# Da-Tsuchi/KLab_MultiModalModel

Measured on AMD Instinct MI355X. Metric: caption-train samples/sec (224px img, 64-tok tgt), higher is better.
Workload: dtype bf16; 1 GPU; BASELINE configs[1]: Swin-V2(C=64,(2,2,6,2),224,w7) frozen + T5-small, fwd+bwd+Adam, T5 dropout 0.1 on, random-init weights; global_batch=64, per_gpu_batch=64, src_len=9, tgt_len=64, parallelism=dp1, hipgraph=False, optimizer=klab.optim.FusedAdam (Adam update of ref/train.py:28, one kernel)

## Files before the change

include/klab_mm.h:

```cpp
#ifndef KLAB_MM_H
#define KLAB_MM_H
#include <stddef.h>
#include <stdint.h>

#ifdef __cplusplus
extern "C" {
#endif

#define KLAB_OK 0
#define KLAB_ERR_UNSUPPORTED (-2)
#define KLAB_ERR_BADARG (-3)

#define KLAB_F32 0
#define KLAB_BF16 1
#define KLAB_FP8 2

#define KLAB_ACT_NONE 0
#define KLAB_ACT_RELU 1
#define KLAB_ACT_GELU 2

#define KLAB_AUX_NONE 0
#define KLAB_AUX_NONZERO 1
#define KLAB_AUX_DGELU 2

// ... 122 lines not shown

#define KLAB_JPEG_GRAY 0
#define KLAB_JPEG_YCC 1
#define KLAB_JPEG_RGB 2
typedef struct klab_jpeg_info {
  int width, height, ncomp, precision, progressive, supported, colour;
  int hmax, vmax, mcus_x, mcus_y;
  int hs[3], vs[3], bw[3], bh[3], tq[3];
  long long coef_blocks;
} klab_jpeg_info;
typedef struct klab_jpeg_item { klab_jpeg_info info; long long coef_block0; long long rgb_off; } klab_jpeg_item;
int klab_jpeg_read_info(const unsigned char* data, size_t n, klab_jpeg_info* info);
int klab_jpeg_entropy_decode(const unsigned char* data, size_t n, short* coefs, unsigned short* qt, klab_jpeg_info* info);
int klab_jpeg_entropy_decode_batch(const unsigned char* const* data, const size_t* sizes, int n, short* const* coefs,
                                   unsigned short* qt, klab_jpeg_info* infos, int* rcs, int n_threads);
size_t klab_jpeg_decode_ws_bytes(const klab_jpeg_item* items, int n);
int klab_jpeg_decode_device(const short* coefs_dev, const unsigned short* qt_dev, const klab_jpeg_item* items,
                            const klab_jpeg_item* items_dev, int n, unsigned char* rgb_dev, void* ws, size_t ws_bytes, void* stream);

int klab_cast_pack(const void* desc_dev, int ndesc, long total4, void* dst, int dtype, void* stream);
int klab_embed_fwd(const long long* ids, int shift_right, int L, int start_id, int pad_id, const float* table, int vocab,
                   float* out, int rows, int d, float drop_p, const uint32_t* seed_dev, uint32_t tag, int* err_flag,
                   void* stream);
int klab_embed_bwd(const long long* ids, int shift_right, int L, int start_id, int pad_id, const float* dh, float* dtable,
                   int vocab, int rows, int d, float drop_p, const uint32_t* seed_dev, uint32_t tag, void* stream);
int klab_relbias_fwd(const float* table, const int* bucket, float* bias, int heads, int Lq, int Lk, void* stream);
int klab_relbias_bwd(const float* dbias, const int* bucket, float* dtable, int heads, int Lq, int Lk, int nbuckets,
                     void* stream);
int klab_ce_count(const long long* labels, int rows, float* inv_n, void* stream);
int klab_ce_fwd(void* logits, long ld, int dtype, const long long* labels, int rows, int V, float* inv_n, float* loss_row,
                float* loss, int write_grad, void* stream);
int klab_im2col_patch(const float* pixels, void* out, int dtype, int B, int Cin, int Himg, int P, void* stream);
int klab_im2col_patch_ld(const float* pixels, void* out, int dtype, int B, int Cin, int Himg, int P, int ldo, void* stream);
int klab_merge_gather(const float* x, void* out, int dtype, int B, int R, int C, void* stream);
int klab_merge_scatter(const float* dmerged, float* dx, int B, int R, int C, void* stream);
int klab_colsum(const void* dy, long ld, int dtype, int M, int N, float* out, void* stream);
int klab_convert(const float* x, void* y, int dtype, long n, float scale, void* stream);
int klab_add_f32(float* y, const float* x, long n, void* stream);

int klab_gelu_fwd(const void* x, void* y, int dtype, long n, void* stream);
int klab_geglu_fwd(const void* ab, long ldab, void* h, long ldh, int dtype, int M, int F, float drop_p, const uint32_t* seed_dev,
                   uint32_t drop_tag, void* stream);
int klab_geglu_bwd(const void* dh, long lddh, const void* ab, long ldab, void* dab, long lddab, int dtype, int M, int F, float drop_p,
                   const uint32_t* seed_dev, uint32_t drop_tag, void* stream);
int klab_swin_proj_ln_fused(const void* x, const float* shortcut, const void* w, const float* b, const float* gamma, const float* beta,
                            float* out, void* outt, int dtype, int M, int C, float eps, void* stream);
int klab_swin_mlp_fused(const void* x, const float* shortcut, const void* w1, const float* b1, const void* w2, const float* b2,
                        const float* gamma, const float* beta, float* out, void* outt, int dtype, int M, int C, float eps,
                        void* stream);
int klab_swin_patch_embed_fused(const float* pixels, const void* w, int ldw, const float* bias, const float* gamma, const float* beta,
                                float* out, void* outt, int dtype, int B, int in_ch, int image_size, int patch, int C, float eps, void* stream);
int klab_swin_linear_ln_fused(const void* x, const float* shortcut, const void* w, const float* bias, const float* gamma,
                              const float* beta, float* out, void* outt, int dtype, int M, int K, int C, float eps, void* stream);
int klab_swin_cpb_bias_bwd(const float* dbias, const float* bias, const int* index, const float* coords, const float* hidden,
                           const float* w0, const float* w2, float* dtable, float* dw0, float* db0, float* dw2, int ntab, int n,
                           int heads, int nhidden, void* stream);
int klab_swin_cpb_bias_bwd_pz(const float* dbias, const float* bias, const int* index, const float* coords, const float* hidden,
                              const float* w0, const float* w2, float* dtable, float* dw0, float* db0, float* dw2, int ntab, int n,
                              int heads, int nhidden, int dtable_zeroed, void* stream);

typedef struct klab_swin_cfg {
  int image_size, patch, in_ch, embed_dim, n_stages;
  int depths[8], heads[8];
  int window;
  int pretrained_window[8];
  int mlp_ratio, qkv_bias;
  float ln_eps;
} klab_swin_cfg;
typedef struct klab_t5_cfg {
  int vocab, d_model, d_kv, n_heads, d_ff, n_layers, n_dec_layers, rel_buckets, rel_max_dist;
  float dropout, ln_eps;
  int start_id, pad_id, scale_decoder_outputs;
  int ffn_gated;
  int tie_lm_head;
} klab_t5_cfg;
typedef struct klab_model_cfg {
  klab_swin_cfg swin;
  klab_t5_cfg lang, main;
  int dtype;
  int train_swin;
} klab_model_cfg;
typedef struct klab_engine klab_engine;

int klab_sizeof_t5_cfg(void);
int klab_sizeof_model_cfg(void);
int klab_sizeof_sample_args(void);
int klab_sizeof_logits_proc_args(void);
int klab_sizeof_gen_cfg(void);
klab_engine* klab_engine_create(const klab_model_cfg* cfg);
void klab_engine_destroy(klab_engine* e);
int klab_engine_num_params(const klab_engine* e, int model);
int klab_engine_param_info(const klab_engine* e, int model, int i, char* name, int name_cap, long* shape4, int* ndim,
                           long* grad_off );
long klab_engine_grad_elems(const klab_engine* e, int model);
int klab_engine_num_buckets(const klab_engine* e, int segment);
int klab_engine_bucket(const klab_engine* e, int segment, int i, long* off, long* len);
int klab_engine_bucket_wait(klab_engine* e, int segment, int i, void* stream);
int klab_engine_set_bucket_events(klab_engine* e, int on);
int klab_engine_segment(const klab_engine* e, int seg, int* model, long* off, long* len);
size_t klab_engine_workspace_bytes(klab_engine* e, int B, int Ls, int Lt);
int klab_engine_bind(klab_engine* e, int B, int Ls, int Lt, void* workspace, size_t ws_bytes, const void* const* swin_params,
                     const void* const* lang_params, const void* const* main_params, float* main_grads, float* swin_grads,
                     const int* lang_bucket, const int* enc_bucket, const int* dec_bucket, const void* const* swin_coords,
                     const void* const* swin_index, void* stream);
int klab_engine_forward(klab_engine* e, const float* pixels, const long long* src_ids, const long long* tgt_ids, int training,
                        uint32_t seed, int want_grad, void* stream);
// ... 118 lines not shown
```

klab_multimodalmodel_amd/_lib.py:

```python
import ctypes as C
import os

HERE = os.path.dirname(os.path.abspath(__file__))
LIB_PATH = os.environ.get("KLAB_LIB", os.path.join(HERE, "libklab_mm.so"))

F32, BF16, FP8 = 0, 1, 2
ACT_NONE, ACT_RELU, ACT_GELU = 0, 1, 2
AUX_NONE, AUX_NONZERO, AUX_DGELU = 0, 1, 2
ERR_UNSUPPORTED, ERR_BADARG = -2, -3

vp, i32, i64, f32, u32 = C.c_void_p, C.c_int, C.c_long, C.c_float, C.c_uint32


class GemmArgs(C.Structure):
    _fields_ = [("M", i32), ("N", i32), ("K", i32), ("dtype", i32),
                ("A", vp), ("lda", i64), ("a_kmajor", i32),
                ("B", vp), ("ldb", i64), ("b_kmajor", i32),
                ("C", vp), ("ldc", i64), ("c_dtype", i32), ("accumulate", i32),
                ("alpha", f32), ("alpha_dev", vp), ("bias", vp), ("act", i32),
                ("aux", vp), ("ldaux", i64), ("aux_mode", i32), ("aux_scale", f32),
                ("residual", vp), ("ldr", i64), ("r_dtype", i32),
                ("drop_p", f32), ("seed_dev", vp), ("drop_tag", u32), ("name_tag", i32), ("atomic_ok", i32)]


# ... 59 lines not shown
class GenCfg(C.Structure):
    _fields_ = [("mode", i32), ("n", i32), ("max_length", i32), ("eos_id", i32), ("pad_id", i32),
                ("temperature", f32), ("top_k", i32), ("top_p", f32), ("seed", C.c_uint64),
                ("length_penalty", f32), ("early_stopping", i32), ("procs", C.POINTER(LogitsProcCfg)), ("want_logprobs", i32)]


SIGNATURES = {
    "klab_version": [],
    "klab_gemm": [C.POINTER(GemmArgs), vp],
    "klab_gemm_probe_enable": [i32],
    "klab_gemm_probe_read": [vp, vp, vp],
    "klab_rmsnorm_fwd": [vp, vp, vp, i32, vp, vp, i32, i32, f32, i32, i32, i32, f32, vp, u32, vp],
    "klab_rmsnorm_bwd": [vp, vp, vp, vp, vp, vp, vp, i32, vp, i32, i32, i32, i32, i32, f32, u32, f32, u32, vp, vp],
    "klab_rmsnorm_bwd_part": [vp, vp, vp, vp, vp, vp, vp, i32, vp, i32, i32, i32, i32, i32, f32, u32, f32, u32, vp, vp],
    "klab_rmsnorm_part_rows": [i32],
    "klab_colpart_reduce": [vp, i64, i32, i32, vp, i32, vp],
    "klab_adam_step": [vp, i32, i64, vp, vp, vp, vp, i32, f32, f32, f32, f32, f32, f32, f32, vp],
    "klab_adam_step_range": [vp, i32, i64, i64, vp, vp, vp, vp, i32, f32, f32, f32, f32, f32, f32, f32, vp],
    "klab_adafactor_plan": [i32, vp, vp, vp, vp, vp],
    "klab_adafactor_step": [vp, i32, i64, i64, vp, vp, vp, vp, vp, vp, i32, f32, f32, f32, f32, f32, f32, f32, f32, f32, i32, vp],
    "klab_layernorm_fwd": [vp, i32, vp, vp, vp, vp, vp, i32, vp, vp, i32, i32, f32, i32, i32, i32, f32, vp, u32, vp],
    "klab_layernorm_bwd": [vp, vp, i32, vp, vp, vp, vp, vp, vp, i32, i32, i32, i32, i32, f32, vp, u32, vp],
    "klab_rmsnorm_fwd_q8": [vp, vp, vp, vp, vp, vp, i32, i32, f32, f32, vp, u32, vp],
    "klab_layernorm_fwd_q8": [vp, vp, vp, vp, vp, vp, vp, vp, vp, vp, i32, i32, f32, vp],
    "klab_gelu_fwd": [vp, vp, i32, i64, vp],
    "klab_gelu_fwd_q8": [vp, vp, vp, vp, i32, i32, vp],
    "klab_geglu_fwd": [vp, i64, vp, i64, i32, i32, i32, f32, vp, u32, vp],
    "klab_geglu_bwd": [vp, i64, vp, i64, vp, i64, i32, i32, i32, f32, vp, u32, vp],
    "klab_layernorm_bwd_bias": [vp, vp, i32, vp, vp, vp, vp, vp, vp, vp, i32, i32, i32, i32, i32, f32, vp, u32, vp],
    "klab_t5_attn_fwd": [C.POINTER(AttnArgs), vp],
    "klab_t5_attn_bwd": [C.POINTER(AttnArgs), vp],
    "klab_t5_attn_fused_fwd": [C.POINTER(AttnFusedArgs), vp],
    "klab_t5_attn_bwd_fused": [C.POINTER(AttnBwdFusedArgs), vp],
    "klab_t5_beam_decode_attn": [i32, vp, i64, vp, vp, i64, i64, i32, vp, i64, vp, i64, vp, i64, i32, i32, i32, i32, vp],
    "klab_beam_topk": [i32, vp, i64, i32, vp, i32, i32, i32, vp, vp, vp, vp, vp],
    "klab_beam_update": [C.POINTER(BeamUpdateArgs), i32, vp],
    "klab_beam_init": [C.POINTER(BeamUpdateArgs), i32, i32, vp],
    "klab_beam_copy_rows": [i32, vp, i64, i32, vp, i64, i32, i32, vp],
    "klab_sample_rows": [C.POINTER(SampleArgs), vp],
    "klab_logits_process_rows": [C.POINTER(LogitsProcArgs), vp],
    "klab_gen_finalize": [vp, i64, vp, i64, i32, i32, i32, i32, f32, i32, vp, vp, vp, vp],
    "klab_sizeof_sample_args": [],
    "klab_sizeof_logits_proc_args": [],
    "klab_sizeof_gen_cfg": [],
    "klab_beam_topk_scores": [vp, i64, i32, vp, i32, i32, i32, vp, vp, vp, vp, vp],
    "klab_dbias_reduce": [vp, i32, vp, i32, i32, i32, i32, vp],
    "klab_swin_mlp_fused": [vp, vp, vp, vp, vp, vp, vp, vp, vp, vp, i32, i32, i32, f32, vp],
    "klab_gemm_grouped": [vp, i32, vp],
    "klab_gemm_fp8": [C.POINTER(GemmArgs), vp, vp, i64, vp],
    "klab_quant_fp8_rows": [vp, i64, i32, i32, vp, i64, vp, vp],
    "klab_quant_fp8_arena": [vp, i32, i64, vp, vp, vp, vp],
    "klab_swin_qkv_attn_fused": [vp, vp, vp, vp, vp, vp, i32, i32, i32, i32, i32, i32, i32, vp],
    "klab_swin_linear_ln_fused": [vp, vp, vp, vp, vp, vp, vp, vp, i32, i32, i32, i32, f32, vp],
    "klab_swin_patch_embed_fused": [vp, vp, i32, vp, vp, vp, vp, vp, i32, i32, i32, i32, i32, i32, f32, vp],
    "klab_swin_proj_ln_fused": [vp, vp, vp, vp, vp, vp, vp, vp, i32, i32, i32, f32, vp],
    "klab_swin_attn_fwd": [C.POINTER(SwinAttnArgs), vp],
    "klab_swin_attn_bwd": [C.POINTER(SwinAttnArgs), vp],
    "klab_swin_attn_bwd_ws_bytes": [i32, i32, i32, i32, i32, i32],
    "klab_swin_cpb_bias": [vp, vp, vp, vp, vp, vp, vp, vp, i32, i32, i32, i32, vp],
    "klab_swin_cpb_table": [vp, vp, vp, vp, vp, vp, vp, i32, i32, i32, vp],
    "klab_swin_cpb_table_bwd": [vp, vp, vp, vp, vp, vp, vp, vp, vp, i32, i32, i32, vp],
    "klab_cast_pack": [vp, i32, i64, vp, i32, vp],
    "klab_embed_fwd": [vp, i32, i32, i32, i32, vp, i32, vp, i32, i32, f32, vp, u32, vp, vp],
    "klab_embed_bwd": [vp, i32, i32, i32, i32, vp, vp, i32, i32, i32, f32, vp, u32, vp],
    "klab_relbias_fwd": [vp, vp, vp, i32, i32, i32, vp],
    "klab_relbias_bwd": [vp, vp, vp, i32, i32, i32, i32, vp],
    "klab_ce_fwd": [vp, i64, i32, vp, i32, i32, vp, vp, vp, i32, vp],
    "klab_ce_count": [vp, i32, vp, vp],
    "klab_im2col_patch": [vp, vp, i32, i32, i32, i32, i32, vp],
    "klab_im2col_patch_ld": [vp, vp, i32, i32, i32, i32, i32, i32, vp],
    "klab_merge_gather": [vp, vp, i32, i32, i32, i32, vp],
    "klab_merge_scatter": [vp, vp, i32, i32, i32, vp],
    "klab_colsum": [vp, i64, i32, i32, i32, vp, vp],
    "klab_convert": [vp, vp, i32, i64, f32, vp],
    "klab_add_f32": [vp, vp, i64, vp],
    "klab_image_preprocess_ws_bytes": [i32, i32, i32],
    "klab_segv_trace_install": [i32],
    "klab_segv_set_context": [C.c_char_p],
    "klab_image_preprocess": [vp, vp, i32, i32, i32, i32, i32, i32, i32, C.c_double, vp, vp, vp, vp, C.c_size_t, vp],
    "klab_jpeg_read_info": [vp, C.c_size_t, vp],
    "klab_jpeg_entropy_decode": [vp, C.c_size_t, vp, vp, vp],
    "klab_jpeg_entropy_decode_batch": [vp, vp, i32, vp, vp, vp, vp, i32],
    "klab_jpeg_decode_ws_bytes": [vp, i32],
    "klab_jpeg_decode_device": [vp, vp, vp, vp, i32, vp, vp, C.c_size_t, vp],
}


class JpegInfo(C.Structure):
    _fields_ = [("width", i32), ("height", i32), ("ncomp", i32), ("precision", i32), ("progressive", i32), ("supported", i32),
                ("colour", i32), ("hmax", i32), ("vmax", i32), ("mcus_x", i32), ("mcus_y", i32), ("hs", i32 * 3), ("vs", i32 * 3),
                ("bw", i32 * 3), ("bh", i32 * 3), ("tq", i32 * 3), ("coef_blocks", C.c_longlong)]


class JpegItem(C.Structure):
    _fields_ = [("info", JpegInfo), ("coef_block0", C.c_longlong), ("rgb_off", C.c_longlong)]

_lib = None


class KlabError(RuntimeError):
    pass


def load():
    global _lib
    if _lib is not None:
# ... 43 lines not shown
```

klab_multimodalmodel_amd/csrc/engine.cpp:

```cpp
#include <hip/hip_runtime.h>
#include <math.h>
#include <stdio.h>
#include <string.h>

#include <string>
#include <vector>

#include "gemm_shared.h"
#include "klab_mm.h"

namespace {

#define RC(x)                 \
  do {                        \
    int rc__ = (x);           \
    if (rc__ != 0) return rc__; \
  } while (0)

struct ParamInfo {
  std::string name;
  std::vector<long> shape;
  long numel = 0;
  long grad_off = -1;
  long warena_off = -1;
// ... 1016 lines not shown
        qrc = klab_swin_qkv_attn_fused(xt, woff(c, P[ix.qw].warena_off), qkvb, q.ctx, q.bias, W[ix.ls], c.dt, B, q.R, q.w, q.shift, q.H, C,
                                       c.ws());
      if (qrc != 0 && qrc != KLAB_ERR_UNSUPPORTED) return qrc;
      if (qrc != 0) {
        RC(linear_fwd(c, xt, M, C, P[ix.qw].warena_off, 3 * C, q.qkv, 3 * C, c.dt, qkvb));
        klab_swin_attn_args a;
        memset(&a, 0, sizeof(a));
        a.dtype = c.dt; a.qkv = q.qkv; a.ctx = q.ctx; a.bias = q.bias; a.bias_table = q.btab; a.logit_scale = W[ix.ls]; a.lse = q.lse;
        a.B = B; a.R = q.R; a.w = q.w; a.shift = q.shift; a.H = q.H; a.C = C;
        a.bwd_ws = e->sattn_ws; a.bwd_ws_bytes = e->sattn_ws_bytes;
        a.v_bias = qkvb ? qkvb + 2 * C : nullptr;
        RC(klab_swin_attn_fwd(&a, c.ws()));
      }
      int prc = KLAB_ERR_UNSUPPORTED;
      if (!e->cfg.train_swin)
        prc = klab_swin_proj_ln_fused(q.ctx, x, woff(c, P[ix.pw].warena_off), W[ix.pb], W[ix.ln1w], W[ix.ln1b], q.h1, q.h1t, c.dt, M, C, s.ln_eps,
                                      c.ws());
      if (prc != 0 && prc != KLAB_ERR_UNSUPPORTED) return prc;
      static const bool fused_lin_ln = klab::env_on("KLAB_SWIN_FUSED_LIN_LN");
      const bool wide_ln = !e->cfg.train_swin && !e->fp8 && fused_lin_ln;
      if (prc != 0 && wide_ln) {
        prc = klab_swin_linear_ln_fused(q.ctx, x, woff(c, P[ix.pw].warena_off), W[ix.pb], W[ix.ln1w], W[ix.ln1b], q.h1, q.h1t, c.dt, M, C, C,
                                        s.ln_eps, c.ws());
        if (prc != 0 && prc != KLAB_ERR_UNSUPPORTED) return prc;
      }
      if (prc != 0) {
        RC(linear_fwd(c, q.ctx, M, C, P[ix.pw].warena_off, C, q.po, C, c.dt, W[ix.pb]));
        RC(ln_fwd_for_linear(c, q.po, W[ix.ln1w], W[ix.ln1b], x, q.h1, q.h1t, q.mean1, q.rstd1, M, C, s.ln_eps));
      }
      if (e->cfg.train_swin) {
        RC(linear_fwd(c, q.h1t, M, C, P[ix.f1w].warena_off, F, q.z, F, c.dt, W[ix.f1b]));
        RC(gelu_fwd_for_linear(c, q.z, q.a, M, F));
      } else {
        const int frc = klab_swin_mlp_fused(q.h1t, q.h1, woff(c, P[ix.f1w].warena_off), W[ix.f1b], woff(c, P[ix.f2w].warena_off), W[ix.f2b],
                                            W[ix.ln2w], W[ix.ln2b], q.h2, q.h2t, c.dt, M, C, s.ln_eps, c.ws());
        if (frc == 0) { x = q.h2; xt = q.h2t; continue; }
        if (frc != KLAB_ERR_UNSUPPORTED) return frc;
        RC(linear_fwd(c, q.h1t, M, C, P[ix.f1w].warena_off, F, q.a, F, c.dt, W[ix.f1b], KLAB_ACT_GELU));
      }
      int f2rc = KLAB_ERR_UNSUPPORTED;
      if (wide_ln)
        f2rc = klab_swin_linear_ln_fused(q.a, q.h1, woff(c, P[ix.f2w].warena_off), W[ix.f2b], W[ix.ln2w], W[ix.ln2b], q.h2, q.h2t, c.dt, M, F, C,
                                         s.ln_eps, c.ws());
      if (f2rc != 0 && f2rc != KLAB_ERR_UNSUPPORTED) return f2rc;
      if (f2rc != 0) {
        RC(linear_fwd(c, q.a, M, F, P[ix.f2w].warena_off, C, q.fo, C, c.dt, W[ix.f2b]));
        RC(ln_fwd_for_linear(c, q.fo, W[ix.ln2w], W[ix.ln2b], q.h1, q.h2, q.h2t, q.mean2, q.rstd2, M, C, s.ln_eps));
      }
      x = q.h2; xt = q.h2t;
    }
    if (st < s.n_stages - 1) {
      const int R = R0 >> st, C = C0 << st;
      const long M2 = (long)B * (R / 2) * (R / 2);
      RC(klab_merge_gather(x, sb.mg, c.dt, B, R, C, c.ws()));
      RC(linear_fwd(c, sb.mg, (int)M2, 4 * C, P[e->si.st[st].redw].warena_off, 2 * C, sb.mo, 2 * C, c.dt));
      RC(klab_layernorm_fwd(sb.mo, c.dt, W[e->si.st[st].mnw], W[e->si.st[st].mnb], nullptr, sb.xm, sb.xmt, c.dt, sb.mmean, sb.mrstd, (int)M2,
                            2 * C, s.ln_eps, 0, 0, 0, 0.f, nullptr, 0, c.ws()));
      x = sb.xm; xt = sb.xmt;
    }
  }
  const int Cl = C0 << (s.n_stages - 1);
  RC(klab_layernorm_fwd(x, KLAB_F32, W[e->si.lnw], W[e->si.lnb], nullptr, e->enc.h[0], nullptr, c.dt, e->sw_fmean, e->sw_frstd,
                        B * e->Nimg, Cl, s.ln_eps, e->Nimg, e->Le, 0, p_in, e->seed_dev, tag_of(STACK_ENC, 0, SITE_IN), c.ws()));
  return 0;
}

int swin_backward(const Ctx& c, const float* dh0, float p_in);

}

extern "C" int klab_sizeof_t5_cfg(void) { return (int)sizeof(klab_t5_cfg); }
extern "C" int klab_sizeof_model_cfg(void) { return (int)sizeof(klab_model_cfg); }
extern "C" int klab_sizeof_sample_args(void) { return (int)sizeof(klab_sample_args); }
extern "C" int klab_sizeof_logits_proc_args(void) { return (int)sizeof(klab_logits_proc_args); }
extern "C" int klab_sizeof_gen_cfg(void) { return (int)sizeof(klab_gen_cfg); }

extern "C" klab_engine* klab_engine_create(const klab_model_cfg* cfg) {
  if (!cfg) return nullptr;
  if (cfg->dtype != KLAB_F32 && cfg->dtype != KLAB_BF16 && cfg->dtype != KLAB_FP8) return nullptr;
  const klab_swin_cfg& s = cfg->swin;
  if (s.n_stages < 1 || s.n_stages > 8 || s.patch <= 0 || s.image_size % s.patch) return nullptr;
  const long Cl = (long)s.embed_dim << (s.n_stages - 1);
  if (Cl != cfg->main.d_model || cfg->lang.d_model != cfg->main.d_model) return nullptr;
  for (const klab_t5_cfg* t : {&cfg->lang, &cfg->main}) {
    if (!t->ffn_gated) continue;
    if (cfg->dtype == KLAB_FP8 || (t->d_ff & 7) || (((long)t->d_ff * t->d_model) & 15)) return nullptr;
  }
  klab_engine* e = new klab_engine();
  e->cfg = *cfg;
  if (cfg->dtype == KLAB_FP8) { e->fp8 = true; e->cfg.dtype = KLAB_BF16; }
  build_swin_params(cfg->swin, e->P[0], e->si);
  build_t5_params(cfg->lang, true, e->P[1], e->li);
  build_t5_params(cfg->main, false, e->P[2], e->mi);
  plan_arenas(e);
  plan_grads(e);
  return e;
}

static void drain_engine(klab_engine* e) {
  if (!e->side && !e->own) return;
  if (e->own) hipStreamSynchronize(e->own);
  if (e->side) hipStreamSynchronize(e->side);
  hipDeviceSynchronize();
}

extern "C" void klab_engine_destroy(klab_engine* e) {
  if (!e) return;
  drain_engine(e);
  for (auto& g : e->gs) if (g.exec) { hipGraphExecDestroy(g.exec); g.exec = nullptr; }
  if (e->ev_fork) hipEventDestroy(e->ev_fork);
// ... 1125 lines not shown
```

klab_multimodalmodel_amd/csrc/swin_lin_ln.hip:

```cpp
#include <stdlib.h>

#include "common.h"
#include "klab_mm.h"

namespace klab {
namespace {

struct LinLnP {
  const bf16_t* x; const float* shortcut; const bf16_t* w; const float* bias; const float* gamma; const float* beta;
  float* out; bf16_t* outt;
  int M, K; float eps;
};

constexpr int LL_S = 4;

template <int N> __device__ __forceinline__ void ll_wait() { asm volatile("s_waitcnt vmcnt(%0)" ::"n"(N) : "memory"); }

template <int C, int BM>
__global__ __launch_bounds__(256, 2) void swin_linear_ln_fused_kernel(LinLnP p) {
  constexpr int S = LL_S, ABYTES = BM * 64, BBYTES = C * 64, SLOT = ABYTES + BBYTES;
  constexpr int LB = C / 64;
  constexpr int AW = BM / 16, RPT = BM / 4;
  constexpr int WN = C / 4, NI = WN / 16;
  constexpr int MI = BM / 16;
  constexpr int PITCH = (C + 4) * 4;
  constexpr int CPR = C / 4;
  static_assert(BM * PITCH + 2 * 4 * BM * 4 <= S * SLOT, "the staged tile and the row statistics alias the ring");
  static_assert(CPR == 64 && (BM == 32 || BM == 64), "copy-out: thread t owns column chunk t & 63 of rows (t >> 6) + 4 i");
  extern __shared__ __attribute__((aligned(16))) char smem[];
  const int tid = threadIdx.x, lane = tid & 63, g = lane >> 4;
  const int wave = __builtin_amdgcn_readfirstlane(tid >> 6);
  const int wn = wave * WN;
  const long bm0 = (long)blockIdx.x * BM;
  const int nt = p.K / 32;

  const int srow = lane >> 2, schunk = (lane & 3) ^ ((lane >> 4) & 3);
  const bf16_t* asrc;
  const bf16_t* bsrc[LB];
  {
    long gr = bm0 + (wave & (AW - 1)) * 16 + srow;
    gr = gr < p.M ? gr : p.M - 1;
    asrc = p.x + gr * p.K + schunk * 8;
  }
#pragma unroll
  for (int i = 0; i < LB; ++i) bsrc[i] = p.w + (long)((wave * LB + i) * 16 + srow) * p.K + schunk * 8;
  auto issue = [&](int t) {
    if (t >= nt) return;
    char* st = smem + (t % S) * SLOT;
    if (wave < AW)
      __builtin_amdgcn_global_load_lds((const __attribute__((address_space(1))) void*)(asrc + (long)t * 32),
                                       (__attribute__((address_space(3))) void*)(st + wave * 1024), 16, 0, 0);
#pragma unroll
    for (int i = 0; i < LB; ++i)
      __builtin_amdgcn_global_load_lds((const __attribute__((address_space(1))) void*)(bsrc[i] + (long)t * 32),
                                       (__attribute__((address_space(3))) void*)(st + ABYTES + (wave * LB + i) * 1024), 16, 0, 0);
  };
  auto frag = [&](const char* img, int f) {
    const int r = f * 16 + (lane & 15);
    return *reinterpret_cast<const bf16x8*>(img + r * 64 + ((g ^ ((r >> 2) & 3)) * 16));
  };

  const int cc = tid & (CPR - 1);
  const f32x4 gm = *reinterpret_cast<const f32x4*>(p.gamma + cc * 4), bt = *reinterpret_cast<const f32x4*>(p.beta + cc * 4);
  f32x4 bb[NI];
#pragma unroll
  for (int j = 0; j < NI; ++j) bb[j] = *reinterpret_cast<const f32x4*>(p.bias + wn + j * 16 + g * 4);

  f32x4 acc[MI][NI];
#pragma unroll
  for (int i = 0; i < MI; ++i)
#pragma unroll
    for (int j = 0; j < NI; ++j) acc[i][j] = f32x4{0.f, 0.f, 0.f, 0.f};

  issue(0);
  issue(1);
  issue(2);
  for (int t = 0; t < nt; ++t) {
    const int young = nt - 1 - t;
    if (wave < AW) {
      if (young >= 2) ll_wait<2 * (LB + 1)>(); else if (young == 1) ll_wait<LB + 1>(); else ll_wait<0>();
    } else {
      if (young >= 2) ll_wait<2 * LB>(); else if (young == 1) ll_wait<LB>(); else ll_wait<0>();
    }
    __builtin_amdgcn_s_barrier();
    const char* As = smem + (t % S) * SLOT;
    const char* Bs = As + ABYTES;
    issue(t + 3);
    bf16x8 af[MI], bf[NI];
#pragma unroll
    for (int i = 0; i < MI; ++i) af[i] = frag(As, i);
#pragma unroll
    for (int j = 0; j < NI; ++j) bf[j] = frag(Bs, (wn >> 4) + j);
#pragma unroll
    for (int i = 0; i < MI; ++i)
#pragma unroll
      for (int j = 0; j < NI; ++j)
        acc[i][j] = __builtin_amdgcn_mfma_f32_16x16x32_bf16(bf[j], af[i], acc[i][j], 0, 0, 0);
  }
  f32x4 sc[RPT];
#pragma unroll
  for (int i = 0; i < RPT; ++i) {
    long m = bm0 + (tid >> 6) + 4 * i;
    m = m < p.M ? m : p.M - 1;
    sc[i] = *reinterpret_cast<const f32x4*>(p.shortcut + m * C + cc * 4);
  }
  __syncthreads();

  float* red = reinterpret_cast<float*>(smem + BM * PITCH);
#pragma unroll
  for (int i = 0; i < MI; ++i) {
    float s = 0.f;
#pragma unroll
    for (int j = 0; j < NI; ++j)
#pragma unroll
      for (int r = 0; r < 4; ++r) { acc[i][j][r] = (float)(bf16_t)(acc[i][j][r] + bb[j][r]); s += acc[i][j][r]; }
    s += __shfl_xor(s, 16, 64); s += __shfl_xor(s, 32, 64);
    if (g == 0) red[wave * BM + i * 16 + (lane & 15)] = s;
  }
  __syncthreads();
  float mean[MI];
#pragma unroll
  for (int i = 0; i < MI; ++i) {
    const int row = i * 16 + (lane & 15);
    mean[i] = (red[0 * BM + row] + red[1 * BM + row] + red[2 * BM + row] + red[3 * BM + row]) * (1.f / C);
    float v = 0.f;
#pragma unroll
    for (int j = 0; j < NI; ++j)
#pragma unroll
      for (int r = 0; r < 4; ++r) { const float d = acc[i][j][r] - mean[i]; v += d * d; }
    v += __shfl_xor(v, 16, 64); v += __shfl_xor(v, 32, 64);
    if (g == 0) red[(4 + wave) * BM + row] = v;
  }
  __syncthreads();
#pragma unroll
  for (int i = 0; i < MI; ++i) {
    const int row = i * 16 + (lane & 15);
    const float var = (red[4 * BM + row] + red[5 * BM + row] + red[6 * BM + row] + red[7 * BM + row]) * (1.f / C);
    const float rstd = rsqrtf(var + p.eps);
#pragma unroll
    for (int j = 0; j < NI; ++j) {
      f32x4 o;
#pragma unroll
      for (int r = 0; r < 4; ++r) o[r] = (acc[i][j][r] - mean[i]) * rstd;
      *reinterpret_cast<f32x4*>(smem + row * PITCH + (wn + j * 16 + g * 4) * 4) = o;
    }
  }
  __syncthreads();
#pragma unroll
  for (int i = 0; i < RPT; ++i) {
    const int row = (tid >> 6) + 4 * i;
    const long m = bm0 + row;
    if (m >= p.M) continue;
    f32x4 v = *reinterpret_cast<const f32x4*>(smem + row * PITCH + cc * 16);
#pragma unroll
    for (int r = 0; r < 4; ++r) v[r] = sc[i][r] + (v[r] * gm[r] + bt[r]);
    *reinterpret_cast<f32x4*>(p.out + m * C + cc * 4) = v;
    if (p.outt) *reinterpret_cast<bf16x4*>(p.outt + m * C + cc * 4) = bf16x4{(bf16_t)v[0], (bf16_t)v[1], (bf16_t)v[2], (bf16_t)v[3]};
  }
}

}
}

extern "C" int klab_swin_linear_ln_fused(const void* x, const float* shortcut, const void* w, const float* bias, const float* gamma,
                                         const float* beta, float* out, void* outt, int dtype, int M, int K, int C, float eps, void* stream) {
  using namespace klab;
  if (!x || !shortcut || !w || !bias || !gamma || !beta || !out) return KLAB_ERR_BADARG;
  if (dtype != KLAB_BF16 || C != 256 || (K & 31) || K < 128 || ((uintptr_t)x & 15) || ((uintptr_t)w & 15)) return KLAB_ERR_UNSUPPORTED;
  if (M <= 0) return KLAB_OK;
  LinLnP p{(const bf16_t*)x, shortcut, (const bf16_t*)w, bias, gamma, beta, out, (bf16_t*)outt, M, K, eps};
#define KLAB_LL(BM_)                                                                                                              \
  {                                                                                                                               \
    const size_t lds = (size_t)LL_S * (BM_ * 64 + 256 * 64);                                                                      \
    const int rc = ensure_dyn_lds(reinterpret_cast<const void*>(swin_linear_ln_fused_kernel<256, BM_>), lds);                     \
    if (rc) return rc;                                                                                                            \
    hipLaunchKernelGGL((swin_linear_ln_fused_kernel<256, BM_>), dim3((unsigned)((M + BM_ - 1) / BM_)), dim3(256), lds, (hipStream_t)stream, p); \
  }
  if (K >= 512) KLAB_LL(64) else KLAB_LL(32)
#undef KLAB_LL
  KLAB_LAUNCH_CHECK();
  return KLAB_OK;
}
```

klab_multimodalmodel_amd/ops.py:

```python
import ctypes as C

import torch

from . import _lib as L


def _seed_ptr(seed):
    return None if seed is None else seed.data_ptr()


def gemm(A, B, C_out, *, M, N, K, a_kmajor=True, b_kmajor=True, lda=None, ldb=None, ldc=None, alpha=1.0,
         alpha_dev=None, bias=None, act=L.ACT_NONE, aux=None, aux_mode=L.AUX_NONE, aux_scale=1.0, residual=None,
         drop_p=0.0, seed=None, tag=0, accumulate=False, atomic_ok=False, name_tag=0):
    lib = L.load()
    a = L.GemmArgs()
    a.atomic_ok, a.name_tag = int(atomic_ok), name_tag
    a.M, a.N, a.K = M, N, K
    a.dtype = L.dtype_code(A.dtype)
    assert B.dtype == A.dtype
    a.A, a.lda, a.a_kmajor = A.data_ptr(), (lda if lda is not None else A.stride(0)), int(a_kmajor)
    a.B, a.ldb, a.b_kmajor = B.data_ptr(), (ldb if ldb is not None else B.stride(0)), int(b_kmajor)
    a.C, a.ldc, a.c_dtype = C_out.data_ptr(), (ldc if ldc is not None else C_out.stride(0)), L.dtype_code(C_out.dtype)
    a.accumulate = int(accumulate)
    a.alpha = alpha
# ... 22 lines not shown

def gemm_fp8(A8, sa, B8, sb, C_out, *, alpha=1.0, bias=None, act=L.ACT_NONE, residual=None, drop_p=0.0, seed=None, tag=0, name_tag=0):
    lib = L.load()
    a = L.GemmArgs()
    a.M, a.K = A8.shape
    a.N = B8.shape[0]
    a.dtype = L.BF16
    a.name_tag = name_tag
    a.A, a.lda, a.a_kmajor = A8.data_ptr(), A8.stride(0), 1
    a.B, a.ldb, a.b_kmajor = B8.data_ptr(), B8.stride(0), 1
    a.C, a.ldc, a.c_dtype = C_out.data_ptr(), C_out.stride(0), L.dtype_code(C_out.dtype)
    a.alpha = alpha
    a.bias = L.ptr(bias)
    a.act = act
    a.residual = L.ptr(residual)
    a.ldr = residual.stride(0) if residual is not None else 0
    a.r_dtype = L.dtype_code(residual.dtype) if residual is not None else 0
    a.drop_p, a.seed_dev, a.drop_tag = drop_p, _seed_ptr(seed), tag
    L.check(lib.klab_gemm_fp8(C.byref(a), sa.data_ptr(), sb.data_ptr(), 1, L.stream_ptr()), "klab_gemm_fp8")
    return C_out


def rmsnorm_fwd(x, w, y=None, y_f32=None, rstd=None, eps=1e-6, grp=0, grp_stride=0, off=0, drop_p=0.0, seed=None, tag=0):
    lib = L.load()
    rows, d = x.shape
    L.check(lib.klab_rmsnorm_fwd(x.data_ptr(), w.data_ptr(), L.ptr(y), L.dtype_code(y.dtype) if y is not None else 0,
                                 L.ptr(y_f32), L.ptr(rstd), rows, d, eps, grp, grp_stride, off, drop_p, _seed_ptr(seed), tag,
                                 L.stream_ptr()), "klab_rmsnorm_fwd")


def rmsnorm_bwd(dy, x, w, rstd, dres=None, dx=None, dxt=None, dw=None, grp=0, grp_stride=0, off=0, p_y=0.0, tag_y=0,
                p_prev=0.0, tag_prev=0, seed=None):
    lib = L.load()
    rows, d = x.shape
    L.check(lib.klab_rmsnorm_bwd(dy.data_ptr(), x.data_ptr(), w.data_ptr(), rstd.data_ptr(), L.ptr(dres), L.ptr(dx), L.ptr(dxt),
                                 L.dtype_code(dxt.dtype) if dxt is not None else 0, L.ptr(dw), rows, d, grp, grp_stride, off,
                                 p_y, tag_y, p_prev, tag_prev, _seed_ptr(seed), L.stream_ptr()), "klab_rmsnorm_bwd")


def layernorm_fwd(y, gamma, beta, shortcut=None, out=None, outt=None, mean=None, rstd=None, eps=1e-5, grp=0, grp_stride=0,
                  off=0, drop_p=0.0, seed=None, tag=0):
    lib = L.load()
    rows, Cc = y.shape
    L.check(lib.klab_layernorm_fwd(y.data_ptr(), L.dtype_code(y.dtype), gamma.data_ptr(), beta.data_ptr(), L.ptr(shortcut),
                                   L.ptr(out), L.ptr(outt), L.dtype_code(outt.dtype) if outt is not None else 0, L.ptr(mean),
                                   L.ptr(rstd), rows, Cc, eps, grp, grp_stride, off, drop_p, _seed_ptr(seed), tag,
                                   L.stream_ptr()), "klab_layernorm_fwd")


def swin_qkv_attn_fused(x, wqkv, bqkv, ctx, bias, logit_scale, *, B, R, w, shift, H, C):
    lib = L.load()
    L.check(lib.klab_swin_qkv_attn_fused(x.data_ptr(), wqkv.data_ptr(), L.ptr(bqkv), ctx.data_ptr(), bias.data_ptr(), logit_scale.data_ptr(),
                                         L.dtype_code(x.dtype), B, R, w, shift, H, C, L.stream_ptr()), "klab_swin_qkv_attn_fused")


def swin_proj_ln_fused(x, shortcut, w, b, gamma, beta, out, outt=None, eps=1e-5):
    lib = L.load()
    M, Cc = x.shape
    L.check(lib.klab_swin_proj_ln_fused(x.data_ptr(), shortcut.data_ptr(), w.data_ptr(), b.data_ptr(), gamma.data_ptr(), beta.data_ptr(),
                                        out.data_ptr(), L.ptr(outt), L.dtype_code(x.dtype), M, Cc, eps, L.stream_ptr()), "klab_swin_proj_ln_fused")


def swin_mlp_fused(x, shortcut, w1, b1, w2, b2, gamma, beta, out, outt=None, eps=1e-5):
    lib = L.load()
    M, Cc = x.shape
    L.check(lib.klab_swin_mlp_fused(x.data_ptr(), shortcut.data_ptr(), w1.data_ptr(), b1.data_ptr(), w2.data_ptr(), b2.data_ptr(),
                                    gamma.data_ptr(), beta.data_ptr(), out.data_ptr(), L.ptr(outt), L.dtype_code(x.dtype), M, Cc, eps,
                                    L.stream_ptr()), "klab_swin_mlp_fused")


def rmsnorm_fwd_q8(x, w, y, rstd, y8, yscale, eps=1e-6):
    lib = L.load()
    rows, d = x.shape
    L.check(lib.klab_rmsnorm_fwd_q8(x.data_ptr(), w.data_ptr(), y.data_ptr(), L.ptr(rstd), y8.data_ptr(), yscale.data_ptr(), rows, d, eps, 0.0,
                                    None, 0, L.stream_ptr()), "klab_rmsnorm_fwd_q8")


def layernorm_fwd_q8(y, gamma, beta, shortcut, out, outt, mean, rstd, o8, oscale, eps=1e-5):
    lib = L.load()
    rows, Cc = y.shape
    L.check(lib.klab_layernorm_fwd_q8(y.data_ptr(), gamma.data_ptr(), beta.data_ptr(), L.ptr(shortcut), L.ptr(out), outt.data_ptr(), L.ptr(mean),
                                      L.ptr(rstd), o8.data_ptr(), oscale.data_ptr(), rows, Cc, eps, L.stream_ptr()), "klab_layernorm_fwd_q8")


def gelu_fwd(z, a):
    lib = L.load()
    L.check(lib.klab_gelu_fwd(z.data_ptr(), a.data_ptr(), L.dtype_code(z.dtype), z.numel(), L.stream_ptr()), "klab_gelu_fwd")


def geglu_fwd(ab, h, drop_p=0.0, seed_dev=None, tag=0):
    lib = L.load()
    M, F = h.shape
    assert ab.shape == (M, 2 * F) and ab.dtype == h.dtype and ab.stride(1) == 1 and h.stride(1) == 1
    L.check(lib.klab_geglu_fwd(ab.data_ptr(), ab.stride(0), h.data_ptr(), h.stride(0), L.dtype_code(h.dtype), M, F, float(drop_p),
                               L.ptr(seed_dev), int(tag), L.stream_ptr()), "klab_geglu_fwd")


def geglu_bwd(dh, ab, dab, drop_p=0.0, seed_dev=None, tag=0):
    lib = L.load()
    M, F = dh.shape
    assert ab.shape == (M, 2 * F) and dab.shape == (M, 2 * F) and ab.dtype == dh.dtype == dab.dtype
    assert ab.stride(1) == 1 and dh.stride(1) == 1 and dab.stride(1) == 1
    L.check(lib.klab_geglu_bwd(dh.data_ptr(), dh.stride(0), ab.data_ptr(), ab.stride(0), dab.data_ptr(), dab.stride(0),
                               L.dtype_code(dh.dtype), M, F, float(drop_p), L.ptr(seed_dev), int(tag), L.stream_ptr()), "klab_geglu_bwd")


# ... 374 lines not shown
```

Baseline: 11710 samples/s.

## Fuse Swin patch-merge gather, reduction linear and LayerNorm into one kernel

For the frozen Swin encoder, patch merging no longer runs three kernels (2x2 gather, reduction GEMM, LayerNorm). A MERGE variant of the fused linear+LN kernel computes the strided 2x2-neighbour addresses directly in its LDS-DMA loads and applies LayerNorm in the epilogue. This removes the materialised gather buffer and the intermediate GEMM output round trips through memory. The fused path does not write the mean/rstd buffers, so it is only taken when Swin is not trained, and it generalises the copy-out mapping to widths of 128 and 512.

```diff
diff --git a/include/klab_mm.h b/include/klab_mm.h
--- a/include/klab_mm.h
+++ b/include/klab_mm.h
@@ -198,6 +198,8 @@
                                 float* out, void* outt, int dtype, int B, int in_ch, int image_size, int patch, int C, float eps, void* stream);
 int klab_swin_linear_ln_fused(const void* x, const float* shortcut, const void* w, const float* bias, const float* gamma,
                               const float* beta, float* out, void* outt, int dtype, int M, int K, int C, float eps, void* stream);
+int klab_swin_merge_fused(const void* xt, const void* wred, const float* gamma, const float* beta, float* out, void* outt, int dtype,
+                          int B, int R, int C, float eps, void* stream);
 int klab_swin_cpb_bias_bwd(const float* dbias, const float* bias, const int* index, const float* coords, const float* hidden,
                            const float* w0, const float* w2, float* dtable, float* dw0, float* db0, float* dw2, int ntab, int n,
                            int heads, int nhidden, void* stream);
diff --git a/klab_multimodalmodel_amd/_lib.py b/klab_multimodalmodel_amd/_lib.py
--- a/klab_multimodalmodel_amd/_lib.py
+++ b/klab_multimodalmodel_amd/_lib.py
@@ -135,6 +135,7 @@
     "klab_quant_fp8_arena": [vp, i32, i64, vp, vp, vp, vp],
     "klab_swin_qkv_attn_fused": [vp, vp, vp, vp, vp, vp, i32, i32, i32, i32, i32, i32, i32, vp],
     "klab_swin_linear_ln_fused": [vp, vp, vp, vp, vp, vp, vp, vp, i32, i32, i32, i32, f32, vp],
+    "klab_swin_merge_fused": [vp, vp, vp, vp, vp, vp, i32, i32, i32, i32, f32, vp],
     "klab_swin_patch_embed_fused": [vp, vp, i32, vp, vp, vp, vp, vp, i32, i32, i32, i32, i32, i32, f32, vp],
     "klab_swin_proj_ln_fused": [vp, vp, vp, vp, vp, vp, vp, vp, i32, i32, i32, f32, vp],
     "klab_swin_attn_fwd": [C.POINTER(SwinAttnArgs), vp],
diff --git a/klab_multimodalmodel_amd/csrc/engine.cpp b/klab_multimodalmodel_amd/csrc/engine.cpp
--- a/klab_multimodalmodel_amd/csrc/engine.cpp
+++ b/klab_multimodalmodel_amd/csrc/engine.cpp
@@ -1092,10 +1092,17 @@
     if (st < s.n_stages - 1) {
       const int R = R0 >> st, C = C0 << st;
       const long M2 = (long)B * (R / 2) * (R / 2);
-      RC(klab_merge_gather(x, sb.mg, c.dt, B, R, C, c.ws()));
-      RC(linear_fwd(c, sb.mg, (int)M2, 4 * C, P[e->si.st[st].redw].warena_off, 2 * C, sb.mo, 2 * C, c.dt));
-      RC(klab_layernorm_fwd(sb.mo, c.dt, W[e->si.st[st].mnw], W[e->si.st[st].mnb], nullptr, sb.xm, sb.xmt, c.dt, sb.mmean, sb.mrstd, (int)M2,
-                            2 * C, s.ln_eps, 0, 0, 0, 0.f, nullptr, 0, c.ws()));
+      int mrc = KLAB_ERR_UNSUPPORTED;
+      if (!e->cfg.train_swin && !e->fp8 && xt)
+        mrc = klab_swin_merge_fused(xt, woff(c, P[e->si.st[st].redw].warena_off), W[e->si.st[st].mnw], W[e->si.st[st].mnb], sb.xm, sb.xmt, c.dt, B,
+                                    R, C, s.ln_eps, c.ws());
+      if (mrc != 0 && mrc != KLAB_ERR_UNSUPPORTED) return mrc;
+      if (mrc != 0) {
+        RC(klab_merge_gather(x, sb.mg, c.dt, B, R, C, c.ws()));
+        RC(linear_fwd(c, sb.mg, (int)M2, 4 * C, P[e->si.st[st].redw].warena_off, 2 * C, sb.mo, 2 * C, c.dt));
+        RC(klab_layernorm_fwd(sb.mo, c.dt, W[e->si.st[st].mnw], W[e->si.st[st].mnb], nullptr, sb.xm, sb.xmt, c.dt, sb.mmean, sb.mrstd, (int)M2,
+                              2 * C, s.ln_eps, 0, 0, 0, 0.f, nullptr, 0, c.ws()));
+      }
       x = sb.xm; xt = sb.xmt;
     }
   }
diff --git a/klab_multimodalmodel_amd/csrc/swin_lin_ln.hip b/klab_multimodalmodel_amd/csrc/swin_lin_ln.hip
--- a/klab_multimodalmodel_amd/csrc/swin_lin_ln.hip
+++ b/klab_multimodalmodel_amd/csrc/swin_lin_ln.hip
@@ -10,23 +10,28 @@
   const bf16_t* x; const float* shortcut; const bf16_t* w; const float* bias; const float* gamma; const float* beta;
   float* out; bf16_t* outt;
   int M, K; float eps;
+  int R;
 };
 
 constexpr int LL_S = 4;
 
 template <int N> __device__ __forceinline__ void ll_wait() { asm volatile("s_waitcnt vmcnt(%0)" ::"n"(N) : "memory"); }
 
-template <int C, int BM>
+template <int C, int BM, bool MERGE = false>
 __global__ __launch_bounds__(256, 2) void swin_linear_ln_fused_kernel(LinLnP p) {
   constexpr int S = LL_S, ABYTES = BM * 64, BBYTES = C * 64, SLOT = ABYTES + BBYTES;
   constexpr int LB = C / 64;
-  constexpr int AW = BM / 16, RPT = BM / 4;
+  constexpr int AW = BM / 16;
   constexpr int WN = C / 4, NI = WN / 16;
   constexpr int MI = BM / 16;
   constexpr int PITCH = (C + 4) * 4;
   constexpr int CPR = C / 4;
+  constexpr int RPP = 256 / CPR, RPT = BM / RPP;
+  constexpr int CS = C / 2;
   static_assert(BM * PITCH + 2 * 4 * BM * 4 <= S * SLOT, "the staged tile and the row statistics alias the ring");
-  static_assert(CPR == 64 && (BM == 32 || BM == 64), "copy-out: thread t owns column chunk t & 63 of rows (t >> 6) + 4 i");
+  static_assert(C % 64 == 0 && CPR <= 256 && 256 % CPR == 0 && BM % RPP == 0 && BM % 16 == 0 && AW <= 4,
+                "copy-out: thread t owns column chunk t % CPR of rows t / CPR + RPP i; x: one LDS-DMA instruction of waves 0 .. AW - 1");
+  static_assert(!MERGE || CS % 32 == 0, "a k-tile never straddles a quarter");
   extern __shared__ __attribute__((aligned(16))) char smem[];
   const int tid = threadIdx.x, lane = tid & 63, g = lane >> 4;
   const int wave = __builtin_amdgcn_readfirstlane(tid >> 6);
@@ -40,15 +45,27 @@
   {
     long gr = bm0 + (wave & (AW - 1)) * 16 + srow;
     gr = gr < p.M ? gr : p.M - 1;
-    asrc = p.x + gr * p.K + schunk * 8;
+    if constexpr (MERGE) {
+      const int R2 = p.R >> 1;
+      const long b = gr / ((long)R2 * R2);
+      const int rem = (int)(gr - b * R2 * R2), y2 = rem / R2, x2 = rem - y2 * R2;
+      asrc = p.x + ((b * p.R + 2 * y2) * p.R + 2 * x2) * CS + schunk * 8;
+    } else {
+      asrc = p.x + gr * p.K + schunk * 8;
+    }
   }
 #pragma unroll
   for (int i = 0; i < LB; ++i) bsrc[i] = p.w + (long)((wave * LB + i) * 16 + srow) * p.K + schunk * 8;
   auto issue = [&](int t) {
     if (t >= nt) return;
     char* st = smem + (t % S) * SLOT;
+    long ak = (long)t * 32;
+    if constexpr (MERGE) {
+      const int q = (t * 32) / CS;
+      ak += (long)((q & 1) * p.R + (q >> 1) - q) * CS;
+    }
     if (wave < AW)
-      __builtin_amdgcn_global_load_lds((const __attribute__((address_space(1))) void*)(asrc + (long)t * 32),
+      __builtin_amdgcn_global_load_lds((const __attribute__((address_space(1))) void*)(asrc + ak),
                                        (__attribute__((address_space(3))) void*)(st + wave * 1024), 16, 0, 0);
 #pragma unroll
     for (int i = 0; i < LB; ++i)
@@ -60,11 +77,11 @@
     return *reinterpret_cast<const bf16x8*>(img + r * 64 + ((g ^ ((r >> 2) & 3)) * 16));
   };
 
-  const int cc = tid & (CPR - 1);
+  const int cc = tid % CPR;
   const f32x4 gm = *reinterpret_cast<const f32x4*>(p.gamma + cc * 4), bt = *reinterpret_cast<const f32x4*>(p.beta + cc * 4);
   f32x4 bb[NI];
 #pragma unroll
-  for (int j = 0; j < NI; ++j) bb[j] = *reinterpret_cast<const f32x4*>(p.bias + wn + j * 16 + g * 4);
+  for (int j = 0; j < NI; ++j) bb[j] = MERGE ? f32x4{0.f, 0.f, 0.f, 0.f} : *reinterpret_cast<const f32x4*>(p.bias + wn + j * 16 + g * 4);
 
   f32x4 acc[MI][NI];
 #pragma unroll
@@ -100,9 +117,9 @@
   f32x4 sc[RPT];
 #pragma unroll
   for (int i = 0; i < RPT; ++i) {
-    long m = bm0 + (tid >> 6) + 4 * i;
+    long m = bm0 + tid / CPR + RPP * i;
     m = m < p.M ? m : p.M - 1;
-    sc[i] = *reinterpret_cast<const f32x4*>(p.shortcut + m * C + cc * 4);
+    sc[i] = MERGE ? f32x4{0.f, 0.f, 0.f, 0.f} : *reinterpret_cast<const f32x4*>(p.shortcut + m * C + cc * 4);
   }
   __syncthreads();
 
@@ -113,7 +130,10 @@
 #pragma unroll
     for (int j = 0; j < NI; ++j)
 #pragma unroll
-      for (int r = 0; r < 4; ++r) { acc[i][j][r] = (float)(bf16_t)(acc[i][j][r] + bb[j][r]); s += acc[i][j][r]; }
+      for (int r = 0; r < 4; ++r) {
+        if constexpr (!MERGE) acc[i][j][r] = (float)(bf16_t)(acc[i][j][r] + bb[j][r]);
+        s += acc[i][j][r];
+      }
     s += __shfl_xor(s, 16, 64); s += __shfl_xor(s, 32, 64);
     if (g == 0) red[wave * BM + i * 16 + (lane & 15)] = s;
   }
@@ -148,12 +168,12 @@
   __syncthreads();
 #pragma unroll
   for (int i = 0; i < RPT; ++i) {
-    const int row = (tid >> 6) + 4 * i;
+    const int row = tid / CPR + RPP * i;
     const long m = bm0 + row;
     if (m >= p.M) continue;
     f32x4 v = *reinterpret_cast<const f32x4*>(smem + row * PITCH + cc * 16);
 #pragma unroll
-    for (int r = 0; r < 4; ++r) v[r] = sc[i][r] + (v[r] * gm[r] + bt[r]);
+    for (int r = 0; r < 4; ++r) v[r] = MERGE ? v[r] * gm[r] + bt[r] : sc[i][r] + (v[r] * gm[r] + bt[r]);
     *reinterpret_cast<f32x4*>(p.out + m * C + cc * 4) = v;
     if (p.outt) *reinterpret_cast<bf16x4*>(p.outt + m * C + cc * 4) = bf16x4{(bf16_t)v[0], (bf16_t)v[1], (bf16_t)v[2], (bf16_t)v[3]};
   }
@@ -168,7 +188,7 @@
   if (!x || !shortcut || !w || !bias || !gamma || !beta || !out) return KLAB_ERR_BADARG;
   if (dtype != KLAB_BF16 || C != 256 || (K & 31) || K < 128 || ((uintptr_t)x & 15) || ((uintptr_t)w & 15)) return KLAB_ERR_UNSUPPORTED;
   if (M <= 0) return KLAB_OK;
-  LinLnP p{(const bf16_t*)x, shortcut, (const bf16_t*)w, bias, gamma, beta, out, (bf16_t*)outt, M, K, eps};
+  LinLnP p{(const bf16_t*)x, shortcut, (const bf16_t*)w, bias, gamma, beta, out, (bf16_t*)outt, M, K, eps, 0};
 #define KLAB_LL(BM_)                                                                                                              \
   {                                                                                                                               \
     const size_t lds = (size_t)LL_S * (BM_ * 64 + 256 * 64);                                                                      \
@@ -181,3 +201,28 @@
   KLAB_LAUNCH_CHECK();
   return KLAB_OK;
 }
+
+extern "C" int klab_swin_merge_fused(const void* xt, const void* wred, const float* gamma, const float* beta, float* out, void* outt,
+                                     int dtype, int B, int R, int C, float eps, void* stream) {
+  using namespace klab;
+  if (!xt || !wred || !gamma || !beta || !out) return KLAB_ERR_BADARG;
+  if (dtype != KLAB_BF16 || (C != 64 && C != 128 && C != 256) || R < 2 || (R & 1) || ((uintptr_t)xt & 15) || ((uintptr_t)wred & 15) ||
+      ((uintptr_t)out & 15) || ((uintptr_t)outt & 7))
+    return KLAB_ERR_UNSUPPORTED;
+  if (B <= 0) return KLAB_OK;
+  const long M2 = (long)B * (R / 2) * (R / 2);
+  if (M2 > 0x7fffffffL) return KLAB_ERR_UNSUPPORTED;
+  LinLnP p{(const bf16_t*)xt, nullptr, (const bf16_t*)wred, nullptr, gamma, beta, out, (bf16_t*)outt, (int)M2, 4 * C, eps, R};
+#define KLAB_MG(N_, BM_)                                                                                                          \
+  {                                                                                                                               \
+    const size_t lds = (size_t)LL_S * (BM_ * 64 + N_ * 64);                                                                       \
+    const int rc = ensure_dyn_lds(reinterpret_cast<const void*>(swin_linear_ln_fused_kernel<N_, BM_, true>), lds);                \
+    if (rc) return rc;                                                                                                            \
+    hipLaunchKernelGGL((swin_linear_ln_fused_kernel<N_, BM_, true>), dim3((unsigned)((M2 + BM_ - 1) / BM_)), dim3(256), lds,      \
+                       (hipStream_t)stream, p);                                                                                   \
+  }
+  if (C == 64) KLAB_MG(128, 64) else if (C == 128) KLAB_MG(256, 64) else KLAB_MG(512, 32)
+#undef KLAB_MG
+  KLAB_LAUNCH_CHECK();
+  return KLAB_OK;
+}
diff --git a/klab_multimodalmodel_amd/ops.py b/klab_multimodalmodel_amd/ops.py
--- a/klab_multimodalmodel_amd/ops.py
+++ b/klab_multimodalmodel_amd/ops.py
@@ -98,6 +98,14 @@
     lib = L.load()
     L.check(lib.klab_swin_qkv_attn_fused(x.data_ptr(), wqkv.data_ptr(), L.ptr(bqkv), ctx.data_ptr(), bias.data_ptr(), logit_scale.data_ptr(),
                                          L.dtype_code(x.dtype), B, R, w, shift, H, C, L.stream_ptr()), "klab_swin_qkv_attn_fused")
+
+
+def swin_merge_fused(xt, wred, gamma, beta, out, outt=None, eps=1e-5):
+    lib = L.load()
+    B, R, R_, Cc = xt.shape
+    assert R == R_
+    L.check(lib.klab_swin_merge_fused(xt.data_ptr(), wred.data_ptr(), gamma.data_ptr(), beta.data_ptr(), out.data_ptr(), L.ptr(outt),
+                                      L.dtype_code(xt.dtype), B, R, Cc, eps, L.stream_ptr()), "klab_swin_merge_fused")
 
 
 def swin_proj_ln_fused(x, shortcut, w, b, gamma, beta, out, outt=None, eps=1e-5):
```

Result: no change. 11820 samples/s, median of 6 (+0.9%).
